# bschrag620/PyRad

Hardware: NVIDIA B200
Metric: line-gridpoint evals/s (higher is better)
Workload: dtype f32

## Files before the change

pyrad_b200/csrc/api.cu:

```cuda
#include "../../include/pyrad_b200.h"

#include <algorithm>
#include <chrono>
#include <cmath>
#include <cstdio>
#include <cstring>
#include <functional>
#include <string>
#include <vector>

#include "common.cuh"
#include "k1_prepass.cuh"
#include "k2_line_sum.cuh"
#include "k2_narrow.cuh"
#include "k2_point.cuh"
#include "k3_stream.cuh"
#include "k4_derived.cuh"
#include "k5_ingest.cuh"
#include "k9_peaks.cuh"
#include <cub/cub.cuh>
#include <thrust/iterator/counting_iterator.h>

using namespace prb;

// ... 118 lines not shown
    DevBuf<double> far_lag2[2];
    float far_delta2[2][K2_FAR_NODES] = {};
    int64_t narrow_wm = 100;
    bool batch_layers = true;
    bool k3_tma = true;
    bool point_kernel = true;
    bool fuse_single = true;
    bool split_tiles = false;
    DevBuf<double> part_sums;
    DevBuf<unsigned int> part_count;
    int64_t rec_budget_mb = 0;
    PeerState peer;
    DevBuf<unsigned int> peer_err;
    IngestScratch ingest;
    DevBuf<int2> tile_bounds_buf[2];
    int tile_bounds_next = 0;
    int extra_launches = 0;
    cudaStream_t copy_stream = nullptr, stream2 = nullptr;
    std::vector<cudaEvent_t> pipe_ev;
    unsigned long long *pin_scal = nullptr;
    DevBuf<unsigned long long> dev_scal;
    unsigned char *blk_h = nullptr;
    size_t blk_cap = 0;
    DevBuf<unsigned char> blk_d;
    K2Layer *ring_h = nullptr;
    DevBuf<K2Layer> ring_d;
    cudaEvent_t ring_ev[RING] = {};
    int ring_next = 0;

    XscTable xsc[K2_MAX_XSC];
// ... 114 lines not shown
    cudaSetDevice(e->device);
    cudaStreamSynchronize(e->stream);
    e->nu0.release(); e->s296.release(); e->gair.release(); e->gself.release();
    e->elower.release(); e->nair.release(); e->delta.release(); e->group.release(); e->einstein_a.release();
    e->idx.release(); e->recA.release(); e->recB.release(); e->recD.release(); e->gp.release(); e->st.release();
    e->out64.release(); e->scratch_a.release(); e->scratch_b.release(); e->scratch_c.release();
    e->scratch_d.release(); e->scratch_w.release();
    e->kmat.release(); e->rad.release(); e->trans.release(); e->fold.release();
    e->flux_layers.release(); e->flux_part.release(); e->flux_out.release(); e->flux_rows.release();
    e->band_part.release(); e->band_out.release(); e->band_tab.release();
    e->k2tab.release(); e->ring_d.release(); e->peer_err.release();
    if (e->blk_h) cudaFreeHost(e->blk_h);
    if (e->read_stage) cudaFreeHost(e->read_stage);
    e->blk_d.release();
    e->ingest.release();
    e->tile_bounds_buf[0].release(); e->tile_bounds_buf[1].release();
    e->far_lag[0].release(); e->far_lag[1].release(); e->far_lag2[0].release(); e->far_lag2[1].release();
    e->dev_scal.release();
    e->part_sums.release(); e->part_count.release();
    e->xsc_rows.release();
    for (auto &x : e->xsc) { x.fx.release(); x.fy.release(); }
    if (e->pin_scal) cudaFreeHost(e->pin_scal);
    for (auto x : e->pipe_ev) cudaEventDestroy(x);
    if (e->copy_stream) cudaStreamDestroy(e->copy_stream);
    if (e->stream2) cudaStreamDestroy(e->stream2);
    if (e->ring_h) { cudaFreeHost(e->ring_h); for (auto x : e->ring_ev) if (x) cudaEventDestroy(x); }
    peer_release(e);
    for (auto x : e->ev) cudaEventDestroy(x);
    cudaStreamDestroy(e->stream);
    delete e;
    return PRB_OK;
// ... 406 lines not shown

static void fill_k1_row(const prb_engine *e, const LayerJob &j, K1Layer &t) {
    const size_t na = (size_t)e->n_alloc;
    t.T = j.T; t.P = j.P;
    t.lc = layer_consts(j.T, j.P, e->res);
    t.scale = j.scale;
    t.scale_dev = j.scale_dev;
    t.wm = (double)j.wm;
    t.gp = j.gp_dev;
    t.recA = e->recA.p + na * j.slot;
    t.recB = e->recB.p + na * j.slot;
    t.recD = e->recD.p + na * j.slot;
    t.st = j.st_dev;
    t.narrow = j.narrow;
    t.pad = 0;
}

static int run_prepass(prb_engine *e, const LayerJob *jobs, int n, DebugOut dbg, int *launches = nullptr) {
    for (int k0 = 0; k0 < n; k0 += K1_MAX_LAYERS) {
        const int m = std::min(n - k0, K1_MAX_LAYERS);
        K1Table &tab = e->k1_host;
        tab.n = m;
        tab.pad = 0;
        int64_t l0 = jobs[k0].l0, l1 = jobs[k0].l1;
        for (int k = 0; k < m; ++k) {
            fill_k1_row(e, jobs[k0 + k], tab.rows[k]);
            l0 = std::min(l0, jobs[k0 + k].l0);
            l1 = std::max(l1, jobs[k0 + k].l1);
        }
        const int64_t kb = l0 & ~int64_t(3);
        const int64_t ke = std::min<int64_t>(l1 + 8, e->n_alloc);
        const int64_t cnt = ke - kb;
        if (cnt > 0) {
            LinesSoA L{e->nu0.p, e->s296.p, e->gair.p, e->gself.p, e->elower.p, e->nair.p, e->delta.p,
                       e->has_group ? e->group.p : nullptr};
            k1_prepass<false><<<(unsigned)((cnt + 255) / 256), 256, 0, e->stream>>>(L, e->idx.p, tab, kb, ke, e->n_lines,
                                                                            e->i_begin, dbg);
            CK(cudaGetLastError());
            if (launches) ++*launches;
            LineRangeTable lr;
            lr.n = 0; lr.pad = 0;
            const size_t na = (size_t)e->n_alloc;
            for (int k = 0; k < m; ++k) {
                const LayerJob &j = jobs[k0 + k];
                if (!j.filter) continue;
                LineRangeRow &r = lr.rows[lr.n++];
                r.recA = e->recA.p + na * j.slot;
                r.recB = e->recB.p + na * j.slot;
                r.recD = e->recD.p + na * j.slot;
                r.lo = j.nu_lo; r.hi = j.nu_hi;
                r.narrow = j.narrow; r.pad = 0;
            }
// ... 58 lines not shown
    CK(cudaMemsetAsync(st.p, 0, sizeof(DevState), e->stream));
    DevBuf<float4> r4, r5; DevBuf<float> r2;
    CK(r4.ensure(na)); CK(r5.ensure(na)); CK(r2.ensure(na));
    K1Table &tab = e->k1_host;
    tab.n = 1;
    K1Layer &row = tab.rows[0];
    row.T = e->last.T; row.P = e->last.P;
    row.lc = layer_consts(e->last.T, e->last.P, e->res);
    row.scale = e->last.scale;
    row.scale_dev = nullptr;
    row.wm = (double)e->last.wm;
    row.gp = e->gp.p;
    row.recA = r4.p; row.recB = r5.p; row.recD = r2.p;
    row.st = st.p;
    row.narrow = 0; row.pad = 0;
    LinesSoA L{e->nu0.p, e->s296.p, e->gair.p, e->gself.p, e->elower.p, e->nair.p, e->delta.p,
               e->has_group ? e->group.p : nullptr};
    k1_prepass<true><<<(unsigned)((na + 255) / 256), 256, 0, e->stream>>>(L, e->idx.p, tab, 0, na, n, e->i_begin, dbg);
    CK(cudaGetLastError());
    if (nu_shift) CK(cudaMemcpyAsync(nu_shift, e->scratch_a.p, sizeof(double) * n, cudaMemcpyDeviceToHost, e->stream));
    if (gamma_l) CK(cudaMemcpyAsync(gamma_l, e->scratch_b.p, sizeof(double) * n, cudaMemcpyDeviceToHost, e->stream));
    if (gamma_d) CK(cudaMemcpyAsync(gamma_d, e->scratch_c.p, sizeof(double) * n, cudaMemcpyDeviceToHost, e->stream));
    if (s_t) CK(cudaMemcpyAsync(s_t, e->scratch_d.p, sizeof(double) * n, cudaMemcpyDeviceToHost, e->stream));
    if (regime) CK(cudaMemcpyAsync(regime, reg.p, sizeof(int32_t) * n, cudaMemcpyDeviceToHost, e->stream));
    std::vector<int32_t> h_idx(index ? n : 0);
    if (index && n) CK(cudaMemcpyAsync(h_idx.data(), e->idx.p, sizeof(int32_t) * n, cudaMemcpyDeviceToHost, e->stream));
    CK(cudaStreamSynchronize(e->stream));
    if (index) for (int64_t i = 0; i < n; ++i) index[i] = h_idx[i];
    r4.release(); r5.release(); r2.release(); reg.release(); st.release();
    return PRB_OK;
// ... 71 lines not shown
    const size_t cnt = (size_t)b.n_layers * b.n_tiles;
    if (e->tile_bounds_buf[e->tile_bounds_next].ensure(cnt) != cudaSuccess)
        return fail(PRB_ERR_CUDA, "tile bounds allocation failed");
    int2 *buf = e->tile_bounds_buf[e->tile_bounds_next].p;
    e->tile_bounds_next ^= 1;
    k2_tile_bounds<<<dim3((unsigned)((b.n_tiles + 255) / 256), (unsigned)b.n_layers), 256, 0, e->stream>>>(
        b.layers, b.n_layers, b.idx, b.i_begin, b.n_tiles, KP_TILE, buf);
    CK(cudaGetLastError());
    ++e->extra_launches;
    b.tile_bounds = buf;
    return PRB_OK;
}

static void xsc_args(const prb_engine *e, K2Args &a);
static int run_line_sum(prb_engine *e, const LayerJob *jobs, int n, const K2Layer *tab_dev, int out_mode,
                        const K2Fuse *fuse, bool with_xsc = false) {
    if (n <= 0) return PRB_OK;
    K2Args a{};
    if (with_xsc) xsc_args(e, a);
    a.layers = tab_dev;
    a.n_layers = n;
    a.idx = e->idx.p;
    a.i_begin = e->i_begin;
    a.n_chunk = (int)chunk_len(e);
    a.variant = e->k2_variant;
    a.out_mode = out_mode;
    a.st = jobs[0].st_dev;
    if (fuse) a.fuse = *fuse;
    cudaError_t ce;
    if (jobs[0].narrow == 2) {
        a.n_tiles = (a.n_chunk + KP_TILE - 1) / KP_TILE;
// ... 11 lines not shown
    }
    if (jobs[0].narrow) {
        a.n_tiles = (a.n_chunk + KN_TILE - 1) / KN_TILE;
        for (int k0 = 0; k0 < n && a.n_tiles > 0; k0 += 65535) {
            K2Args b = a;
            b.layers = tab_dev + k0;
            b.n_layers = std::min(n - k0, 65535);
            int rc2 = tile_bounds(e, b);
            if (rc2) return rc2;
            k2_narrow<<<dim3((unsigned)a.n_tiles, (unsigned)b.n_layers), KN_THREADS, sizeof(KNSmem), e->stream>>>(b);
        }
        ce = cudaGetLastError();
        if (ce != cudaSuccess) return fail(PRB_ERR_CUDA, std::string("k2_narrow launch failed: ") + cudaGetErrorString(ce));
        return PRB_OK;
    }
    switch (jobs[0].ppt) {
        case 2: ce = launch_k2_t<2>(e, a); break;
        case 4: ce = launch_k2_t<4>(e, a); break;
        case 16: ce = launch_k2_t<16>(e, a); break;
        default: ce = launch_k2_t<8>(e, a); break;
    }
    if (ce != cudaSuccess) return fail(PRB_ERR_CUDA, std::string("k2_line_sum launch failed: ") + cudaGetErrorString(ce));
    return PRB_OK;
}

extern "C" int prb_line_sum_dev(prb_engine *e, void *out_dev, int out_mode) {
    if (!e) return fail(PRB_ERR_ARG, "null engine");
    if (!e->last.valid) return fail(PRB_ERR_STATE, "prb_line_sum: run prb_layer_prepass first");
    if (!e->seg.empty()) return fail(PRB_ERR_STATE, "prb_line_sum: grouped line list -- use prb_line_sum_groups");
    if (!out_dev) return fail(PRB_ERR_ARG, "prb_line_sum_dev: NULL output");
// ... 482 lines not shown
        for (int sidx = 0; sidx < pipe->S; ++sidx) {
            if (sidx + 1 < pipe->S && (rc = pipe->enqueue_piece(sidx + 1))) return rc;
            cudaStream_t st = (sidx & 1) ? pipe->stream2 : e->stream;
            CK(cudaStreamWaitEvent(st, pipe->ev[sidx], 0));
            if (sidx) CK(cudaStreamWaitEvent(st, pipe->ev_k1[sidx - 1], 0));
            const int64_t a = sidx ? pipe->line_hi[sidx - 1] : 0;
            const int64_t b = sidx == pipe->S - 1 ? na : pipe->line_hi[sidx];
            if (b > a) {
                k0_line_index<<<(unsigned)((b - a + 255) / 256), 256, 0, st>>>(e->nu0.p, n, a, b, e->range_min, e->res, e->idx.p);
                CK(cudaGetLastError());
                LayerJob jj = jobs[0];
                jj.l0 = a;
                jj.l1 = std::min<int64_t>(b, n);
                K1Table &tab = e->k1_host;
                tab.n = 1;
                tab.pad = 0;
                fill_k1_row(e, jj, tab.rows[0]);
                LinesSoA Ls{e->nu0.p, e->s296.p, e->gair.p, e->gself.p, e->elower.p, e->nair.p, e->delta.p,
                            e->has_group ? e->group.p : nullptr};
                k1_prepass<false><<<(unsigned)((b - a + 255) / 256), 256, 0, st>>>(Ls, e->idx.p, tab, a, b, n, e->i_begin, DebugOut{});
                CK(cudaGetLastError());
                launches += 2;
            }
            CK(cudaEventRecord(pipe->ev_k1[sidx], st));
            K2Args ka{};
            ka.layers = k2_dev + sidx;
            ka.n_layers = 1;
            ka.idx = e->idx.p;
            ka.i_begin = e->i_begin;
            ka.n_chunk = (int)nc;
            ka.variant = e->k2_variant;
// ... 7 lines not shown
            switch (jobs[0].ppt) {
                case 2: ce = launch_k2_sub<2>(e, ka, st); break;
                case 4: ce = launch_k2_sub<4>(e, ka, st); break;
                case 16: ce = launch_k2_sub<16>(e, ka, st); break;
                default: ce = launch_k2_sub<8>(e, ka, st); break;
            }
            if (ce != cudaSuccess) return fail(PRB_ERR_CUDA, std::string("k2_line_sum sub-launch failed: ") + cudaGetErrorString(ce));
            ++launches;
        }
        CK(cudaEventRecord(pipe->ev_k1[pipe->S], pipe->stream2));
        CK(cudaStreamWaitEvent(e->stream, pipe->ev_k1[pipe->S], 0));
    }
    for (int bi = 0; bi < (pipe ? 0 : n_batches); ++bi) {
        const int b0 = (int)(bi * slots), b1 = (int)std::min<int64_t>(n_layers, b0 + slots);
        if (e->timing) CK(cudaEventRecord(e->ev[3 * bi], e->stream));
        rc = run_prepass(e, jobs.data() + b0, b1 - b0, DebugOut{}, &launches);
        if (rc) return rc;
        if (e->timing) CK(cudaEventRecord(e->ev[3 * bi + 1], e->stream));
        for (int c0 = b0; c0 < b1;) {
            int c1 = c0 + 1;
            while (c1 < b1 && jobs[c1].narrow == jobs[c0].narrow && (jobs[c0].narrow || jobs[c1].ppt == jobs[c0].ppt)) ++c1;
            rc = run_line_sum(e, jobs.data() + c0, c1 - c0, k2_dev + c0, PRB_OUT_F32, fused ? &fuse : nullptr, true);
            if (rc) return rc;
            ++launches;
            c0 = c1;
        }
        if (e->timing) CK(cudaEventRecord(e->ev[3 * bi + 2], e->stream));
    }
    if (e->timing) CK(cudaEventRecord(e->ev[3 * n_batches], e->stream));
    if (nc > 0 && !fused) {
        if (e->k3_tma && n_layers >= K3T_LAYERS) {
            const int64_t n_strips = (nc + K3T_STRIP - 1) / K3T_STRIP;
            const int grid = (int)std::min<int64_t>(n_strips, K3T_MINB * (int64_t)e->prop.multiProcessorCount);
            double t_max = t_surface, t_min = t_surface;
            for (int l = 0; l < n_layers; ++l) { t_max = std::max(t_max, t_layer[l]); t_min = std::min(t_min, t_layer[l]); }
            double nu_min = std::max(3 * dx * std::sqrt(6.0 / 8e-7), 0.26 * t_max / c2);
            if ((3 * dx) * (3 * dx) / 8 * (c2 / t_min) * (c2 / t_min) > 1e-7) nu_min = 1e30;
// ... 887 lines not shown
```

pyrad_b200/csrc/common.cuh:

```cuda
#pragma once
#include <cuda_runtime.h>
#include <stdint.h>
#include <math.h>

namespace prb {

constexpr double kBoltz = 1.38064852E-23;
constexpr double cLight = 299792458.0;
constexpr double hPlanck = 6.62607004e-34;
constexpr double kPi = 3.141592653589793;
constexpr double kT0 = 296.0;
constexpr double kP0 = 1013.25;
constexpr double kAvogadro = 6.022140857E23;

constexpr int REGIME_GAUSS = 0, REGIME_LORENTZ = 1, REGIME_VOIGT = 2;

struct GroupParams {
    double conc;
    double dopp;
    double qratio;
    double weight;
};

struct DevState {
    unsigned int reserved0;
    unsigned int flags;
    unsigned int tile_counter;
    unsigned int pad;
};

constexpr unsigned int FLAG_OVERFLOW = 1u, FLAG_NONFINITE = 2u;

#ifndef PRB_K2_CONSUMERS
#define PRB_K2_CONSUMERS 8
#endif
#ifndef PRB_K2_ACC_SMEM
#define PRB_K2_ACC_SMEM 0
#endif
constexpr int K2_CONSUMERS = PRB_K2_CONSUMERS;
constexpr int K2_THREADS = 32 * (K2_CONSUMERS + 1);
#ifndef PRB_K2_CHUNK
#define PRB_K2_CHUNK 768
#endif
#ifndef PRB_K2_STAGES
#define PRB_K2_STAGES 3
#endif
#ifndef PRB_K2_MIN_CTAS
#define PRB_K2_MIN_CTAS 2
#endif
constexpr int K2_CHUNK = PRB_K2_CHUNK;
constexpr int K2_STAGES = PRB_K2_STAGES;
constexpr int K2_MIN_CTAS = PRB_K2_MIN_CTAS;
constexpr int K2_FLUSH = 64;
constexpr float K2_SENTINEL = 3.0e38f;

__device__ __forceinline__ uint32_t smem_u32(const void *p) {
    return (uint32_t)__cvta_generic_to_shared(p);
}
__device__ __forceinline__ void mbar_init(uint64_t *bar, uint32_t count) {
    asm volatile("mbarrier.init.shared::cta.b64 [%0], %1;" ::"r"(smem_u32(bar)), "r"(count) : "memory");
}
__device__ __forceinline__ void mbar_expect_tx(uint64_t *bar, uint32_t bytes) {
    asm volatile("mbarrier.arrive.expect_tx.shared::cta.b64 _, [%0], %1;" ::"r"(smem_u32(bar)), "r"(bytes)
                 : "memory");
}
__device__ __forceinline__ void mbar_arrive(uint64_t *bar) {
    asm volatile("mbarrier.arrive.shared::cta.b64 _, [%0];" ::"r"(smem_u32(bar)) : "memory");
}
__device__ __forceinline__ void mbar_wait(uint64_t *bar, uint32_t parity) {
    asm volatile(
        "{\n"
        ".reg .pred p;\n"
        "WAIT_%=:\n"
        "mbarrier.try_wait.parity.shared::cta.b64 p, [%0], %1;\n"
        "@p bra DONE_%=;\n"
        "bra WAIT_%=;\n"
        "DONE_%=:\n"
        "}\n" ::"r"(smem_u32(bar)),
        "r"(parity)
        : "memory");
}
__device__ __forceinline__ void mbar_wait_parked(uint64_t *bar, uint32_t parity) {
    asm volatile(
        "{\n"
        ".reg .pred p;\n"
        "WAITP_%=:\n"
        "mbarrier.try_wait.parity.shared::cta.b64 p, [%0], %1, %2;\n"
        "@p bra DONEP_%=;\n"
        "bra WAITP_%=;\n"
        "DONEP_%=:\n"
        "}\n" ::"r"(smem_u32(bar)),
        "r"(parity), "r"(4000u)
        : "memory");
}
__device__ __forceinline__ void tma_bulk_g2s(void *dst, const void *src, uint32_t bytes, uint64_t *bar) {
    asm volatile(
        "cp.async.bulk.shared::cluster.global.mbarrier::complete_tx::bytes [%0], [%1], %2, [%3];" ::"r"(
            smem_u32(dst)),
        "l"(src), "r"(bytes), "r"(smem_u32(bar))
        : "memory");
}

}
```

pyrad_b200/csrc/k1_prepass.cuh:

```cuda
#pragma once
#include "common.cuh"

namespace prb {

struct LinesSoA {
    const double *nu0, *s296, *gair, *gself, *elower, *nair, *delta;
    const int32_t *group;
};

struct LayerConsts {
    double log_t0_over_t;
    double inv_t_minus_inv_t0;
    double inv_res2;
    double res2;
    double p_over_p0;
    double neg_c2_over_t;
    double neg_c2_over_t0;
};

struct DebugOut {
    double *nu_shift, *gl, *gd, *st;
    int32_t *regime;
};

// ... 72 lines not shown

__device__ __forceinline__ double pow5(double x) { double x2 = x * x; return x2 * x2 * x; }

struct K1Layer {
    double T, P;
    LayerConsts lc;
    double scale;
    const double *scale_dev;
    double wm;
    const GroupParams *gp;
    float4 *recA, *recB;
    float *recD;
    DevState *st;
    int narrow;
    int pad;
};

constexpr int K1_MAX_LAYERS = 128;
enum K1Const {
    K1C_EXP_INV = 0, K1C_EXP_MAGIC, K1C_EXP_HI, K1C_EXP_LO, K1C_EXP_5, K1C_EXP_4, K1C_EXP_3,
    K1C_T7, K1C_T6, K1C_T5, K1C_T4, K1C_T3,
    K1C_V1, K1C_V2, K1C_V3, K1C_V4,
    K1C_E1, K1C_E2, K1C_E3,
    K1C_LOG2E, K1C_INV_SQRTPI, K1C_INV_PI, K1C_FIFTH, K1C_C2, K1C_NEG_C2_T0,
    K1C_LO_A, K1C_LO_B, K1C_HI_A, K1C_HI_B,
    K1C_BIG, K1C_COUNT
};
struct K1Table {
    int n;
    int pad;
    double c[K1C_COUNT];
    K1Layer rows[K1_MAX_LAYERS];
};
inline void k1_fill_constants(K1Table &t) {
    const double eps = 1e-14, c2 = cLight * hPlanck * 100 / kBoltz;
    const double v[K1C_COUNT] = {
        92.33248261689366, 6755399441055744.0, -0.01083042469326756, -2.9815858269852933e-12, 1.0 / 120.0, 1.0 / 24.0, 1.0 / 6.0,
        1.0 / 5040, 1.0 / 720, 1.0 / 120, 1.0 / 24, 1.0 / 6,
        2.69269, 2.42843, 4.47163, .07842,
        1.36603, .47719, .11116,
        1.4426950408889634, 0.5641895835477563, 1.0 / kPi, 0.2, c2, -c2 / kT0,
        .01 * (1 - eps), .01 * (1 + eps), 100 * (1 + eps), 100 * (1 - eps),
        8.0e37};
    for (int i = 0; i < K1C_COUNT; ++i) t.c[i] = v[i];
}
// ... 54 lines not shown
    p = fma(p, x, c[K1C_T5]);
    p = fma(p, x, c[K1C_T4]);
    p = fma(p, x, c[K1C_T3]);
    p = fma(p, x, 0.5);
    p = fma(p, x, 1.0);
    return fma(p, x, 1.0);
}

#ifndef PRB_K1_UNROLL
#define PRB_K1_UNROLL 1
#endif
constexpr int K1_UNROLL = PRB_K1_UNROLL;
#ifndef PRB_K1_MINB
#define PRB_K1_MINB 4
#endif
template <bool DEBUG = false>
__global__ void __launch_bounds__(256, PRB_K1_MINB)
k1_prepass(LinesSoA L, const int32_t *__restrict__ idx, const __grid_constant__ K1Table tab,
           int64_t l_begin, int64_t l_end, int64_t n_lines, int64_t i_base, DebugOut dbg) {
    __shared__ double exp_tab[64];
    if (threadIdx.x < 64) exp_tab[threadIdx.x] = K1_EXP_TAB[threadIdx.x];
    __syncthreads();
    const double *__restrict__ cst = tab.c;
    const double c2 = cst[K1C_C2];
    const int64_t l = l_begin + (int64_t)blockIdx.x * blockDim.x + threadIdx.x;
    const bool in_range = l < l_end;
    const bool real = in_range && l < n_lines && !(L.group && L.group[l] < 0);
    double nu = 0, delta = 0, gair = 0, gself = 0, nair = 0, elower = 0, s296 = 0;
    float nf = 0.f;
    int g = 0;
    if (real) {
        nu = L.nu0[l]; delta = L.delta[l]; gair = L.gair[l]; gself = L.gself[l];
        nair = L.nair[l]; elower = L.elower[l]; s296 = L.s296[l];
        g = L.group ? L.group[l] : 0;
        nf = -(float)((double)((int64_t)idx[l] - i_base));
    }
    const bool bad_line = real && !isfinite(nu + delta + gair + gself + nair + elower + s296);
    const double e296 = exp_k1(cst[K1C_NEG_C2_T0] * nu, exp_tab, cst);
    const double neg_c2_e = -c2 * elower;
    const int n_layers = tab.n;
// ... 149 lines not shown
```

pyrad_b200/csrc/k2_line_sum.cuh:

```cuda
#pragma once
#include "common.cuh"
#include "k3_stream.cuh"

namespace prb {

__device__ __forceinline__ float rcp_approx(float x) {
    float r;
    asm("rcp.approx.ftz.f32 %0, %1;" : "=f"(r) : "f"(x));
    return r;
}
__device__ __forceinline__ float ex2_approx(float x) {
    float r;
    asm("ex2.approx.ftz.f32 %0, %1;" : "=f"(r) : "f"(x));
    return r;
}

__device__ __forceinline__ void tma_bulk_s2g(void *dst, const void *src, uint32_t bytes) {
    asm volatile("cp.async.bulk.global.shared::cta.bulk_group [%0], [%1], %2;" ::"l"(dst), "r"(smem_u32(src)), "r"(bytes)
                 : "memory");
}
__device__ __forceinline__ void consumer_barrier() {
    asm volatile("bar.sync 1, %0;" ::"n"(K2_CONSUMERS * 32) : "memory");
}

__device__ __forceinline__ int warp_lower_bound(const int32_t *__restrict__ idx, int lo, int hi, long long key) {
    const int lane = threadIdx.x & 31;
    while (hi > lo) {
        const int span = hi - lo;
        const int step = (span + 31) >> 5;
        int pos = lo + (lane + 1) * step - 1;
        pos = pos < hi - 1 ? pos : hi - 1;
        const bool less = (long long)__ldg(idx + pos) < key;
        const unsigned m = __ballot_sync(0xffffffffu, less);
        const int c = __popc(m);
        int nlo = lo, nhi = hi;
        if (c > 0) { int p = lo + c * step - 1; p = p < hi - 1 ? p : hi - 1; nlo = p + 1; }
        if (c < 32) { int p = lo + (c + 1) * step - 1; p = p < hi - 1 ? p : hi - 1; nhi = p; }
        lo = nlo;
        hi = nhi;
    }
    return lo;
}

constexpr int K2_MAX_XSC = 8;
struct K2Layer {
    const float4 *recA;
    const float4 *recB;
    const float *recD;
    void *out;
    double inv_scale;
    int l_begin, l_end;
    int wm;
    int pad;
    double xsc_w[K2_MAX_XSC];
};

// ... 7 lines not shown
    long long n_total;
    double x0, dx, x_last;
    float *rad[K2_MAX_DST];
    float *trans[K2_MAX_DST];
};

struct K2Args {
    const K2Layer *layers;
    int n_layers;
    const int32_t *idx;
    long long i_begin;
    int n_chunk;
    int n_tiles;
    int tile_base;
    const int2 *tile_bounds;
    int variant;
    int out_mode;
    DevState *st;
    K2Fuse fuse;
    const double *far_lag;
    float far_delta[16];
    const double *far_lag2;
    float far_delta2[16];
    const double *xsc_sigma;
    long long xsc_ld;
    int n_xsc;
    int parts;
    double *part_sums;
    unsigned int *part_count;
};
// ... 16 lines not shown
#define PRB_K2_FAR2_ENABLE 1
#endif
constexpr bool K2_FAR2 = PRB_K2_FAR2_ENABLE != 0;
constexpr int K2_FAR2_MIN_DOMAINS = 4;
static_assert(K2_CONSUMERS % K2_FAR2_SPANS == 0, "a tile is a whole number of level-2 domains");

struct K2Desc {
    int tile0;
    int cnt;
    int flags;
    int layer;
    int part;
};
constexpr int K2_FIRST = 1, K2_LAST = 2, K2_END = 4;

struct K2Smem {
    float4 rA[K2_STAGES][K2_CHUNK];
    float4 rB[K2_STAGES][K2_CHUNK];
    float rD[K2_STAGES][K2_CHUNK];
    K2Desc desc[K2_STAGES];
    uint64_t full[K2_STAGES];
    uint64_t empty[K2_STAGES];
    double far2[2][K2_CONSUMERS][K2_FAR_NODES];
    double2 faracc[2][K2_CONSUMERS * 32];
    int part_last;
};

template <int P>
__host__ __device__ constexpr size_t K2_SMEM_BASE() {
    return ((sizeof(K2Smem) + (PRB_K2_ACC_SMEM ? sizeof(double) * P * K2_CONSUMERS * 32 : 0)) + 127) & ~size_t(127);
}
template <int P>
__host__ __device__ constexpr size_t K2_SMEM_BYTES(bool peer_staging) {
    return K2_SMEM_BASE<P>() + (peer_staging ? sizeof(float) * 2 * K2_CONSUMERS * 32 * P : 0);
}

template <int H>
// ... 227 lines not shown
#pragma unroll
            for (int h = 0; h < H; ++h) {
                const float ex = s.fi[h].x + a.x, ey = s.fi[h].y + a.x;
                const float e2x = ex * ex, e2y = ey * ey;
                float tx = a.z * rcp_approx(e2x + b.x), ty = a.z * rcp_approx(e2y + b.x);
                tx = fmaf(b.z, ex2_approx(b.w * e2x), tx);
                ty = fmaf(b.z, ex2_approx(b.w * e2y), ty);
                s.a32[h].x += (fabsf(ex) <= wmf) ? tx : 0.f;
                s.a32[h].y += (fabsf(ey) <= wmf) ? ty : 0.f;
            }
        }
        s.flush();
    }
}

template <int P, bool FAR, bool SPLIT>
__device__ __forceinline__ void k2_line_sum_body(const K2Args &a) {
    static_assert(P >= 2 && P % 2 == 0, "points per thread must be even (packed FP32x2)");
    static_assert(!FAR || P == 4 || P == 8, "far-field tables exist for 128- and 256-point spans");
    constexpr int H = P / 2;
    constexpr int TILE = K2_CONSUMERS * 32 * P;
    constexpr int SPAN = 32 * P;
    extern __shared__ __align__(128) unsigned char smem_raw[];
    K2Smem &sm = *reinterpret_cast<K2Smem *>(smem_raw);
    const int tid = threadIdx.x, lane = tid & 31, warp = tid >> 5;

    if (tid == 0) {
        for (int s = 0; s < K2_STAGES; ++s) {
            mbar_init(&sm.full[s], 1);
            mbar_init(&sm.empty[s], K2_CONSUMERS);
        }
        asm volatile("fence.mbarrier_init.release.cluster;" ::: "memory");
        asm volatile("fence.proxy.async.shared::cta;" ::: "memory");
    }
    __syncthreads();

    if (warp == K2_CONSUMERS) {
        uint32_t it = 0;
        auto slot_acquire = [&](uint32_t &stage) {
            stage = it % K2_STAGES;
            mbar_wait_parked(&sm.empty[stage], ((it / K2_STAGES) & 1) ^ 1);
        };
        const int parts = (SPLIT && a.parts > 1) ? a.parts : 1;
        const int n_items = a.n_layers * a.n_tiles * parts;
        while (true) {
            int item = 0;
            if (lane == 0) item = (int)atomicAdd(&a.st->tile_counter, 1u);
            item = __shfl_sync(0xffffffffu, item, 0);
            if (item >= n_items) break;
            const int n_lt = a.n_layers * a.n_tiles;
            const int pidx = item / n_lt;
            const int lt = item - pidx * n_lt;
            const int half = parts >> 1, step = pidx >> 2, r = pidx & 3;
            const int part = parts < 4 ? pidx : (r == 0 ? half - 1 - step : r == 1 ? half + step : r == 2 ? step : parts - 1 - step);
            const int layer = lt / a.n_tiles;
            const int tile = a.tile_base + lt - layer * a.n_tiles;
            const K2Layer *L = a.layers + layer;
            const int wm = __ldg(&L->wm), l_begin = __ldg(&L->l_begin), l_end = __ldg(&L->l_end);
            const float4 *recA = L->recA;
            const float4 *recB = L->recB;
            const float *recD = L->recD;
            const int tile0 = tile * TILE;
            const long long k_lo = a.i_begin + tile0 - wm;
            const long long k_hi = a.i_begin + tile0 + TILE - 1 + wm + 1;
            int lo = warp_lower_bound(a.idx, l_begin, l_end, k_lo);
            const int hi = warp_lower_bound(a.idx, lo, l_end, k_hi);
            lo &= ~3;
            const int nch = hi > lo ? (hi - lo + K2_CHUNK - 1) / K2_CHUNK : 1;
            const int c0 = (int)((long long)part * nch / parts), c1 = (int)((long long)(part + 1) * nch / parts);
            const int cn = c1 > c0 ? c1 - c0 : 1;
            for (int k = 0; k < cn; ++k, ++it) {
                const int c = c0 + k;
                uint32_t stage;
                slot_acquire(stage);
                if (lane == 0) {
                    const int first = lo + c * K2_CHUNK;
                    const int cnt = c1 > c0 ? max(min(K2_CHUNK, hi - first), 0) : 0;
                    sm.desc[stage] = K2Desc{tile0, cnt, (k == 0 ? K2_FIRST : 0) | (k == cn - 1 ? K2_LAST : 0), layer, part};
                    if (cnt > 0) {
                        const uint32_t ce = (uint32_t)((cnt + 3) & ~3);
                        mbar_expect_tx(&sm.full[stage], ce * 36u);
                        tma_bulk_g2s(sm.rA[stage], recA + first, ce * 16u, &sm.full[stage]);
                        tma_bulk_g2s(sm.rB[stage], recB + first, ce * 16u, &sm.full[stage]);
                        tma_bulk_g2s(sm.rD[stage], recD + first, ce * 4u, &sm.full[stage]);
                    } else {
                        mbar_arrive(&sm.full[stage]);
                    }
                }
                __syncwarp();
            }
        }
        uint32_t stage;
        slot_acquire(stage);
        if (lane == 0) {
            sm.desc[stage] = K2Desc{0, 0, K2_END, 0, 0};
            mbar_arrive(&sm.full[stage]);
        }
        return;
    }

    float wmf = 0.f;
    Acc<H> s;
#pragma unroll
    for (int h = 0; h < H; ++h) { s.a32[h] = make_float2(0.f, 0.f); s.fi[h] = make_float2(0.f, 0.f); }
#if PRB_K2_ACC_SMEM
    s.a64 = reinterpret_cast<double *>(smem_raw + sizeof(K2Smem)) + tid;
#endif
#pragma unroll
    for (int p = 0; p < P; ++p) s.acc(p) = 0.0;
    int wb = 0;
    float wbf = 0.f, we1f = 0.f;
    double2 *far = &sm.faracc[0][tid];
    double2 *far2 = &sm.faracc[1][tid];
    float dbf = 0.f;
// ... 108 lines not shown
                b4 = __reduce_add_sync(0xffffffffu, c4);
                const int b5 = __reduce_add_sync(0xffffffffu, c5);
                bg0 = __reduce_add_sync(0xffffffffu, cg0);
                bg1 = __reduce_add_sync(0xffffffffu, cg1);
                lorentz_paired<H, true>(sA, sB, b0, b1, wmf, s);
                lorentz_paired<H, false>(sA, sB, b1, b4, wmf, s);
                lorentz_paired<H, true>(sA, sB, b4, b5, wmf, s);
            }
            if (dgmax > 0.f) {
                gauss_pass<H, true>(sA, sB, sD, bg0, min(bg1, b1), wbf, we1f, wmf, s);
                gauss_pass<H, false>(sA, sB, sD, max(bg0, b1), min(bg1, b4), wbf, we1f, wmf, s);
                gauss_pass<H, true>(sA, sB, sD, max(bg0, b4), bg1, wbf, we1f, wmf, s);
            }
        }
        __syncwarp();
        if (lane == 0) mbar_arrive(&sm.empty[stage]);

        if (d.flags & K2_LAST) {
            const K2Layer *L = a.layers + d.layer;
            const double inv_scale = __ldg(&L->inv_scale);
            void *out = L->out;
            const bool bulk = a.fuse.enabled && a.fuse.n_dst > 1 && d.tile0 + TILE <= a.n_chunk;
            float *stage_rad = reinterpret_cast<float *>(smem_raw + K2_SMEM_BASE<P>());
            float *stage_tr = stage_rad + TILE;
            if (bulk) {
                if (tid == 0) asm volatile("cp.async.bulk.wait_group.read 0;" ::: "memory");
                consumer_barrier();
            }
            if (FAR) {
                double v0 = far->x, v1 = far->y, w0 = far2->x, w1 = far2->y;
#pragma unroll
// ... 113 lines not shown
```

Baseline: 4989 billion.

## Remove dedicated producer warp and precompute tile line bounds in prepass

Drops the dedicated TMA producer warp from the line-sum kernel. The last consumer warp to release a stage now refills it, with shared-memory counters and an ordered issue ticket replacing the empty mbarriers. Per-tile line-index bounds for wide layers are computed by extra blocks of the prepass kernel and stored in a device buffer, so the refill path reads them instead of doing a warp binary search. This frees a warp per CTA and takes the search off the critical path, but refill latency now lands on consumer warps and the spin on the issue counter can serialize them.

Measured after the change: 5056 billion (median of 6 runs). 1.4% higher.

```diff
diff --git a/pyrad_b200/csrc/api.cu b/pyrad_b200/csrc/api.cu
--- a/pyrad_b200/csrc/api.cu
+++ b/pyrad_b200/csrc/api.cu
@@ -156,6 +156,7 @@
     DevBuf<unsigned int> peer_err;
     IngestScratch ingest;
     DevBuf<int2> tile_bounds_buf[2];
+    DevBuf<int2> k2_bounds;
     int tile_bounds_next = 0;
     int extra_launches = 0;
     cudaStream_t copy_stream = nullptr, stream2 = nullptr;
@@ -300,7 +301,7 @@
     if (e->read_stage) cudaFreeHost(e->read_stage);
     e->blk_d.release();
     e->ingest.release();
-    e->tile_bounds_buf[0].release(); e->tile_bounds_buf[1].release();
+    e->tile_bounds_buf[0].release(); e->tile_bounds_buf[1].release(); e->k2_bounds.release();
     e->far_lag[0].release(); e->far_lag[1].release(); e->far_lag2[0].release(); e->far_lag2[1].release();
     e->dev_scal.release();
     e->part_sums.release(); e->part_count.release();
@@ -737,28 +738,43 @@
     t.st = j.st_dev;
     t.narrow = j.narrow;
     t.pad = 0;
-}
-
-static int run_prepass(prb_engine *e, const LayerJob *jobs, int n, DebugOut dbg, int *launches = nullptr) {
+    t.bounds = nullptr;
+    t.b_tiles = t.b_tile_pts = t.b_l_begin = t.b_l_end = t.b_wm = 0;
+}
+
+static int run_prepass(prb_engine *e, const LayerJob *jobs, int n, DebugOut dbg, int *launches = nullptr,
+                       int2 *bounds = nullptr, int64_t bounds_ld = 0) {
+    const int64_t nc = chunk_len(e);
     for (int k0 = 0; k0 < n; k0 += K1_MAX_LAYERS) {
         const int m = std::min(n - k0, K1_MAX_LAYERS);
         K1Table &tab = e->k1_host;
         tab.n = m;
-        tab.pad = 0;
+        tab.bounds_blocks = 0;
         int64_t l0 = jobs[k0].l0, l1 = jobs[k0].l1;
         for (int k = 0; k < m; ++k) {
-            fill_k1_row(e, jobs[k0 + k], tab.rows[k]);
-            l0 = std::min(l0, jobs[k0 + k].l0);
-            l1 = std::max(l1, jobs[k0 + k].l1);
+            const LayerJob &j = jobs[k0 + k];
+            K1Layer &r = tab.rows[k];
+            fill_k1_row(e, j, r);
+            l0 = std::min(l0, j.l0);
+            l1 = std::max(l1, j.l1);
+            if (bounds && !j.narrow) {
+                r.bounds = bounds + (size_t)(k0 + k) * bounds_ld;
+                r.b_tile_pts = K2_CONSUMERS * 32 * j.ppt;
+                r.b_tiles = (int)((nc + r.b_tile_pts - 1) / r.b_tile_pts);
+                r.b_l_begin = (int)j.l0;
+                r.b_l_end = (int)j.l1;
+                r.b_wm = (int)j.wm;
+                tab.bounds_blocks = std::max(tab.bounds_blocks, (r.b_tiles + 7) / 8);
+            }
         }
         const int64_t kb = l0 & ~int64_t(3);
-        const int64_t ke = std::min<int64_t>(l1 + 8, e->n_alloc);
+        const int64_t ke = std::max(kb, std::min<int64_t>(l1 + 8, e->n_alloc));
         const int64_t cnt = ke - kb;
-        if (cnt > 0) {
+        if (cnt > 0 || tab.bounds_blocks > 0) {
             LinesSoA L{e->nu0.p, e->s296.p, e->gair.p, e->gself.p, e->elower.p, e->nair.p, e->delta.p,
                        e->has_group ? e->group.p : nullptr};
-            k1_prepass<false><<<(unsigned)((cnt + 255) / 256), 256, 0, e->stream>>>(L, e->idx.p, tab, kb, ke, e->n_lines,
-                                                                            e->i_begin, dbg);
+            const int64_t blocks = (cnt + 255) / 256 + (int64_t)m * tab.bounds_blocks;
+            k1_prepass<false><<<(unsigned)blocks, 256, 0, e->stream>>>(L, e->idx.p, tab, kb, ke, e->n_lines, e->i_begin, dbg);
             CK(cudaGetLastError());
             if (launches) ++*launches;
             LineRangeTable lr;
@@ -847,6 +863,8 @@
     row.recA = r4.p; row.recB = r5.p; row.recD = r2.p;
     row.st = st.p;
     row.narrow = 0; row.pad = 0;
+    row.bounds = nullptr;
+    tab.bounds_blocks = 0;
     LinesSoA L{e->nu0.p, e->s296.p, e->gair.p, e->gself.p, e->elower.p, e->nair.p, e->delta.p,
                e->has_group ? e->group.p : nullptr};
     k1_prepass<true><<<(unsigned)((na + 255) / 256), 256, 0, e->stream>>>(L, e->idx.p, tab, 0, na, n, e->i_begin, dbg);
@@ -948,7 +966,8 @@
 
 static void xsc_args(const prb_engine *e, K2Args &a);
 static int run_line_sum(prb_engine *e, const LayerJob *jobs, int n, const K2Layer *tab_dev, int out_mode,
-                        const K2Fuse *fuse, bool with_xsc = false) {
+                        const K2Fuse *fuse, bool with_xsc = false, const int2 *wide_bounds = nullptr,
+                        int64_t bounds_ld = 0) {
     if (n <= 0) return PRB_OK;
     K2Args a{};
     if (with_xsc) xsc_args(e, a);
@@ -990,6 +1009,8 @@
         if (ce != cudaSuccess) return fail(PRB_ERR_CUDA, std::string("k2_narrow launch failed: ") + cudaGetErrorString(ce));
         return PRB_OK;
     }
+    a.tile_bounds = wide_bounds;
+    a.bounds_ld = (int)bounds_ld;
     switch (jobs[0].ppt) {
         case 2: ce = launch_k2_t<2>(e, a); break;
         case 4: ce = launch_k2_t<4>(e, a); break;
@@ -1502,7 +1523,7 @@
                 jj.l1 = std::min<int64_t>(b, n);
                 K1Table &tab = e->k1_host;
                 tab.n = 1;
-                tab.pad = 0;
+                tab.bounds_blocks = 0;
                 fill_k1_row(e, jj, tab.rows[0]);
                 LinesSoA Ls{e->nu0.p, e->s296.p, e->gair.p, e->gself.p, e->elower.p, e->nair.p, e->delta.p,
                             e->has_group ? e->group.p : nullptr};
@@ -1540,13 +1561,16 @@
     for (int bi = 0; bi < (pipe ? 0 : n_batches); ++bi) {
         const int b0 = (int)(bi * slots), b1 = (int)std::min<int64_t>(n_layers, b0 + slots);
         if (e->timing) CK(cudaEventRecord(e->ev[3 * bi], e->stream));
-        rc = run_prepass(e, jobs.data() + b0, b1 - b0, DebugOut{}, &launches);
+        const int64_t bounds_ld = (nc + 511) / 512;
+        CK(e->k2_bounds.ensure((size_t)std::max<int64_t>(bounds_ld, 1) * (b1 - b0)));
+        rc = run_prepass(e, jobs.data() + b0, b1 - b0, DebugOut{}, &launches, e->k2_bounds.p, bounds_ld);
         if (rc) return rc;
         if (e->timing) CK(cudaEventRecord(e->ev[3 * bi + 1], e->stream));
         for (int c0 = b0; c0 < b1;) {
             int c1 = c0 + 1;
             while (c1 < b1 && jobs[c1].narrow == jobs[c0].narrow && (jobs[c0].narrow || jobs[c1].ppt == jobs[c0].ppt)) ++c1;
-            rc = run_line_sum(e, jobs.data() + c0, c1 - c0, k2_dev + c0, PRB_OUT_F32, fused ? &fuse : nullptr, true);
+            rc = run_line_sum(e, jobs.data() + c0, c1 - c0, k2_dev + c0, PRB_OUT_F32, fused ? &fuse : nullptr, true,
+                              e->k2_bounds.p + (size_t)(c0 - b0) * bounds_ld, bounds_ld);
             if (rc) return rc;
             ++launches;
             c0 = c1;
diff --git a/pyrad_b200/csrc/common.cuh b/pyrad_b200/csrc/common.cuh
--- a/pyrad_b200/csrc/common.cuh
+++ b/pyrad_b200/csrc/common.cuh
@@ -38,7 +38,7 @@
 #define PRB_K2_ACC_SMEM 0
 #endif
 constexpr int K2_CONSUMERS = PRB_K2_CONSUMERS;
-constexpr int K2_THREADS = 32 * (K2_CONSUMERS + 1);
+constexpr int K2_THREADS = 32 * K2_CONSUMERS;
 #ifndef PRB_K2_CHUNK
 #define PRB_K2_CHUNK 768
 #endif
@@ -53,6 +53,25 @@
 constexpr int K2_MIN_CTAS = PRB_K2_MIN_CTAS;
 constexpr int K2_FLUSH = 64;
 constexpr float K2_SENTINEL = 3.0e38f;
+
+__device__ __forceinline__ int warp_lower_bound(const int32_t *__restrict__ idx, int lo, int hi, long long key) {
+    const int lane = threadIdx.x & 31;
+    while (hi > lo) {
+        const int span = hi - lo;
+        const int step = (span + 31) >> 5;
+        int pos = lo + (lane + 1) * step - 1;
+        pos = pos < hi - 1 ? pos : hi - 1;
+        const bool less = (long long)__ldg(idx + pos) < key;
+        const unsigned m = __ballot_sync(0xffffffffu, less);
+        const int c = __popc(m);
+        int nlo = lo, nhi = hi;
+        if (c > 0) { int p = lo + c * step - 1; p = p < hi - 1 ? p : hi - 1; nlo = p + 1; }
+        if (c < 32) { int p = lo + (c + 1) * step - 1; p = p < hi - 1 ? p : hi - 1; nhi = p; }
+        lo = nlo;
+        hi = nhi;
+    }
+    return lo;
+}
 
 __device__ __forceinline__ uint32_t smem_u32(const void *p) {
     return (uint32_t)__cvta_generic_to_shared(p);
@@ -80,19 +99,6 @@
         "r"(parity)
         : "memory");
 }
-__device__ __forceinline__ void mbar_wait_parked(uint64_t *bar, uint32_t parity) {
-    asm volatile(
-        "{\n"
-        ".reg .pred p;\n"
-        "WAITP_%=:\n"
-        "mbarrier.try_wait.parity.shared::cta.b64 p, [%0], %1, %2;\n"
-        "@p bra DONEP_%=;\n"
-        "bra WAITP_%=;\n"
-        "DONEP_%=:\n"
-        "}\n" ::"r"(smem_u32(bar)),
-        "r"(parity), "r"(4000u)
-        : "memory");
-}
 __device__ __forceinline__ void tma_bulk_g2s(void *dst, const void *src, uint32_t bytes, uint64_t *bar) {
     asm volatile(
         "cp.async.bulk.shared::cluster.global.mbarrier::complete_tx::bytes [%0], [%1], %2, [%3];" ::"r"(
diff --git a/pyrad_b200/csrc/k1_prepass.cuh b/pyrad_b200/csrc/k1_prepass.cuh
--- a/pyrad_b200/csrc/k1_prepass.cuh
+++ b/pyrad_b200/csrc/k1_prepass.cuh
@@ -110,6 +110,9 @@
     DevState *st;
     int narrow;
     int pad;
+    int2 *bounds;
+    int b_tiles, b_tile_pts;
+    int b_l_begin, b_l_end, b_wm;
 };
 
 constexpr int K1_MAX_LAYERS = 128;
@@ -124,7 +127,7 @@
 };
 struct K1Table {
     int n;
-    int pad;
+    int bounds_blocks;
     double c[K1C_COUNT];
     K1Layer rows[K1_MAX_LAYERS];
 };
@@ -209,16 +212,31 @@
 #ifndef PRB_K1_MINB
 #define PRB_K1_MINB 4
 #endif
+__device__ __noinline__ void k1_tile_bounds(const K1Table &tab, const int32_t *__restrict__ idx, int64_t i_base, int b) {
+    const K1Layer &R = tab.rows[b / tab.bounds_blocks];
+    const int t = (b % tab.bounds_blocks) * 8 + (int)(threadIdx.x >> 5);
+    if (!R.bounds || t >= R.b_tiles) return;
+    const long long tile0 = i_base + (long long)t * R.b_tile_pts;
+    const int lo = warp_lower_bound(idx, R.b_l_begin, R.b_l_end, tile0 - R.b_wm);
+    const int hi = warp_lower_bound(idx, lo, R.b_l_end, tile0 + R.b_tile_pts - 1 + R.b_wm + 1);
+    if ((threadIdx.x & 31) == 0) R.bounds[t] = make_int2(lo, hi);
+}
+
 template <bool DEBUG = false>
 __global__ void __launch_bounds__(256, PRB_K1_MINB)
 k1_prepass(LinesSoA L, const int32_t *__restrict__ idx, const __grid_constant__ K1Table tab,
            int64_t l_begin, int64_t l_end, int64_t n_lines, int64_t i_base, DebugOut dbg) {
+    const int bounds_blocks = tab.n * tab.bounds_blocks;
+    if ((int)blockIdx.x < bounds_blocks) {
+        k1_tile_bounds(tab, idx, i_base, (int)blockIdx.x);
+        return;
+    }
     __shared__ double exp_tab[64];
     if (threadIdx.x < 64) exp_tab[threadIdx.x] = K1_EXP_TAB[threadIdx.x];
     __syncthreads();
     const double *__restrict__ cst = tab.c;
     const double c2 = cst[K1C_C2];
-    const int64_t l = l_begin + (int64_t)blockIdx.x * blockDim.x + threadIdx.x;
+    const int64_t l = l_begin + (int64_t)(blockIdx.x - bounds_blocks) * blockDim.x + threadIdx.x;
     const bool in_range = l < l_end;
     const bool real = in_range && l < n_lines && !(L.group && L.group[l] < 0);
     double nu = 0, delta = 0, gair = 0, gself = 0, nair = 0, elower = 0, s296 = 0;
diff --git a/pyrad_b200/csrc/k2_line_sum.cuh b/pyrad_b200/csrc/k2_line_sum.cuh
--- a/pyrad_b200/csrc/k2_line_sum.cuh
+++ b/pyrad_b200/csrc/k2_line_sum.cuh
@@ -21,25 +21,6 @@
 }
 __device__ __forceinline__ void consumer_barrier() {
     asm volatile("bar.sync 1, %0;" ::"n"(K2_CONSUMERS * 32) : "memory");
-}
-
-__device__ __forceinline__ int warp_lower_bound(const int32_t *__restrict__ idx, int lo, int hi, long long key) {
-    const int lane = threadIdx.x & 31;
-    while (hi > lo) {
-        const int span = hi - lo;
-        const int step = (span + 31) >> 5;
-        int pos = lo + (lane + 1) * step - 1;
-        pos = pos < hi - 1 ? pos : hi - 1;
-        const bool less = (long long)__ldg(idx + pos) < key;
-        const unsigned m = __ballot_sync(0xffffffffu, less);
-        const int c = __popc(m);
-        int nlo = lo, nhi = hi;
-        if (c > 0) { int p = lo + c * step - 1; p = p < hi - 1 ? p : hi - 1; nlo = p + 1; }
-        if (c < 32) { int p = lo + (c + 1) * step - 1; p = p < hi - 1 ? p : hi - 1; nhi = p; }
-        lo = nlo;
-        hi = nhi;
-    }
-    return lo;
 }
 
 constexpr int K2_MAX_XSC = 8;
@@ -77,6 +58,7 @@
     int n_tiles;
     int tile_base;
     const int2 *tile_bounds;
+    int bounds_ld;
     int variant;
     int out_mode;
     DevState *st;
@@ -123,13 +105,23 @@
 };
 constexpr int K2_FIRST = 1, K2_LAST = 2, K2_END = 4;
 
+struct K2Cursor {
+    int layer, part, tile0;
+    int lo, hi;
+    int c0, c1;
+    int k, cn;
+    int done;
+};
+
 struct K2Smem {
     float4 rA[K2_STAGES][K2_CHUNK];
     float4 rB[K2_STAGES][K2_CHUNK];
     float rD[K2_STAGES][K2_CHUNK];
     K2Desc desc[K2_STAGES];
     uint64_t full[K2_STAGES];
-    uint64_t empty[K2_STAGES];
+    unsigned int released[K2_STAGES];
+    unsigned int issued;
+    K2Cursor cur;
     double far2[2][K2_CONSUMERS][K2_FAR_NODES];
     double2 faracc[2][K2_CONSUMERS * 32];
     int part_last;
@@ -387,6 +379,78 @@
     }
 }
 
+struct K2Item {
+    int part, layer, tile;
+};
+__device__ __forceinline__ K2Item k2_item(const K2Args &a, int item, int parts) {
+    const int n_lt = a.n_layers * a.n_tiles;
+    const int pidx = item / n_lt;
+    const int lt = item - pidx * n_lt;
+    const int half = parts >> 1, step = pidx >> 2, r = pidx & 3;
+    const int part = parts < 4 ? pidx : (r == 0 ? half - 1 - step : r == 1 ? half + step : r == 2 ? step : parts - 1 - step);
+    const int layer = lt / a.n_tiles;
+    return K2Item{part, layer, a.tile_base + lt - layer * a.n_tiles};
+}
+
+template <int TILE, bool SPLIT>
+__device__ __forceinline__ void k2_refill(K2Smem &sm, const K2Args &a, uint32_t stage) {
+    const int lane = threadIdx.x & 31;
+    K2Cursor c = sm.cur;
+    if (c.done) return;
+    if (c.k == c.cn) {
+        const int parts = (SPLIT && a.parts > 1) ? a.parts : 1;
+        int item = 0;
+        if (lane == 0) item = (int)atomicAdd(&a.st->tile_counter, 1u);
+        item = __shfl_sync(0xffffffffu, item, 0);
+        if (item >= a.n_layers * a.n_tiles * parts) {
+            if (lane == 0) {
+                sm.desc[stage] = K2Desc{0, 0, K2_END, 0, 0};
+                mbar_arrive(&sm.full[stage]);
+                sm.cur.done = 1;
+            }
+            __syncwarp();
+            return;
+        }
+        const K2Item w = k2_item(a, item, parts);
+        const int tile0 = w.tile * TILE;
+        int lo, hi;
+        if (a.tile_bounds) {
+            const int2 bd = __ldg(a.tile_bounds + (size_t)w.layer * a.bounds_ld + (w.tile - a.tile_base));
+            lo = bd.x;
+            hi = bd.y;
+        } else {
+            const K2Layer *L = a.layers + w.layer;
+            const int wm = __ldg(&L->wm), l_begin = __ldg(&L->l_begin), l_end = __ldg(&L->l_end);
+            const long long k_lo = a.i_begin + tile0 - wm;
+            const long long k_hi = a.i_begin + tile0 + TILE - 1 + wm + 1;
+            lo = warp_lower_bound(a.idx, l_begin, l_end, k_lo);
+            hi = warp_lower_bound(a.idx, lo, l_end, k_hi);
+        }
+        lo &= ~3;
+        const int nch = hi > lo ? (hi - lo + K2_CHUNK - 1) / K2_CHUNK : 1;
+        const int c0 = (int)((long long)w.part * nch / parts), c1 = (int)((long long)(w.part + 1) * nch / parts);
+        c = K2Cursor{w.layer, w.part, tile0, lo, hi, c0, c1, 0, c1 > c0 ? c1 - c0 : 1, 0};
+    }
+    if (lane == 0) {
+        const int first = c.lo + (c.c0 + c.k) * K2_CHUNK;
+        const int cnt = c.c1 > c.c0 ? max(min(K2_CHUNK, c.hi - first), 0) : 0;
+        sm.desc[stage] = K2Desc{c.tile0, cnt, (c.k == 0 ? K2_FIRST : 0) | (c.k == c.cn - 1 ? K2_LAST : 0), c.layer, c.part};
+        if (cnt > 0) {
+            const K2Layer *L = a.layers + c.layer;
+            const uint32_t ce = (uint32_t)((cnt + 3) & ~3);
+            mbar_expect_tx(&sm.full[stage], ce * 36u);
+            tma_bulk_g2s(sm.rA[stage], L->recA + first, ce * 16u, &sm.full[stage]);
+            tma_bulk_g2s(sm.rB[stage], L->recB + first, ce * 16u, &sm.full[stage]);
+            tma_bulk_g2s(sm.rD[stage], L->recD + first, ce * 4u, &sm.full[stage]);
+        } else {
+            mbar_arrive(&sm.full[stage]);
+        }
+        ++c.k;
+        sm.cur = c;
+    }
+    __syncwarp();
+}
+
 template <int P, bool FAR, bool SPLIT>
 __device__ __forceinline__ void k2_line_sum_body(const K2Args &a) {
     static_assert(P >= 2 && P % 2 == 0, "points per thread must be even (packed FP32x2)");
@@ -398,79 +462,21 @@
     K2Smem &sm = *reinterpret_cast<K2Smem *>(smem_raw);
     const int tid = threadIdx.x, lane = tid & 31, warp = tid >> 5;
 
-    if (tid == 0) {
-        for (int s = 0; s < K2_STAGES; ++s) {
-            mbar_init(&sm.full[s], 1);
-            mbar_init(&sm.empty[s], K2_CONSUMERS);
-        }
-        asm volatile("fence.mbarrier_init.release.cluster;" ::: "memory");
-        asm volatile("fence.proxy.async.shared::cta;" ::: "memory");
+    if (warp == 0) {
+        if (lane == 0) {
+            for (int s = 0; s < K2_STAGES; ++s) {
+                mbar_init(&sm.full[s], 1);
+                sm.released[s] = 0;
+            }
+            sm.issued = K2_STAGES;
+            sm.cur = K2Cursor{0, 0, 0, 0, 0, 0, 0, 0, 0, 0};
+            asm volatile("fence.mbarrier_init.release.cluster;" ::: "memory");
+            asm volatile("fence.proxy.async.shared::cta;" ::: "memory");
+        }
+        __syncwarp();
+        for (int s = 0; s < K2_STAGES; ++s) k2_refill<TILE, SPLIT>(sm, a, s);
     }
     __syncthreads();
-
-    if (warp == K2_CONSUMERS) {
-        uint32_t it = 0;
-        auto slot_acquire = [&](uint32_t &stage) {
-            stage = it % K2_STAGES;
-            mbar_wait_parked(&sm.empty[stage], ((it / K2_STAGES) & 1) ^ 1);
-        };
-        const int parts = (SPLIT && a.parts > 1) ? a.parts : 1;
-        const int n_items = a.n_layers * a.n_tiles * parts;
-        while (true) {
-            int item = 0;
-            if (lane == 0) item = (int)atomicAdd(&a.st->tile_counter, 1u);
-            item = __shfl_sync(0xffffffffu, item, 0);
-            if (item >= n_items) break;
-            const int n_lt = a.n_layers * a.n_tiles;
-            const int pidx = item / n_lt;
-            const int lt = item - pidx * n_lt;
-            const int half = parts >> 1, step = pidx >> 2, r = pidx & 3;
-            const int part = parts < 4 ? pidx : (r == 0 ? half - 1 - step : r == 1 ? half + step : r == 2 ? step : parts - 1 - step);
-            const int layer = lt / a.n_tiles;
-            const int tile = a.tile_base + lt - layer * a.n_tiles;
-            const K2Layer *L = a.layers + layer;
-            const int wm = __ldg(&L->wm), l_begin = __ldg(&L->l_begin), l_end = __ldg(&L->l_end);
-            const float4 *recA = L->recA;
-            const float4 *recB = L->recB;
-            const float *recD = L->recD;
-            const int tile0 = tile * TILE;
-            const long long k_lo = a.i_begin + tile0 - wm;
-            const long long k_hi = a.i_begin + tile0 + TILE - 1 + wm + 1;
-            int lo = warp_lower_bound(a.idx, l_begin, l_end, k_lo);
-            const int hi = warp_lower_bound(a.idx, lo, l_end, k_hi);
-            lo &= ~3;
-            const int nch = hi > lo ? (hi - lo + K2_CHUNK - 1) / K2_CHUNK : 1;
-            const int c0 = (int)((long long)part * nch / parts), c1 = (int)((long long)(part + 1) * nch / parts);
-            const int cn = c1 > c0 ? c1 - c0 : 1;
-            for (int k = 0; k < cn; ++k, ++it) {
-                const int c = c0 + k;
-                uint32_t stage;
-                slot_acquire(stage);
-                if (lane == 0) {
-                    const int first = lo + c * K2_CHUNK;
-                    const int cnt = c1 > c0 ? max(min(K2_CHUNK, hi - first), 0) : 0;
-                    sm.desc[stage] = K2Desc{tile0, cnt, (k == 0 ? K2_FIRST : 0) | (k == cn - 1 ? K2_LAST : 0), layer, part};
-                    if (cnt > 0) {
-                        const uint32_t ce = (uint32_t)((cnt + 3) & ~3);
-                        mbar_expect_tx(&sm.full[stage], ce * 36u);
-                        tma_bulk_g2s(sm.rA[stage], recA + first, ce * 16u, &sm.full[stage]);
-                        tma_bulk_g2s(sm.rB[stage], recB + first, ce * 16u, &sm.full[stage]);
-                        tma_bulk_g2s(sm.rD[stage], recD + first, ce * 4u, &sm.full[stage]);
-                    } else {
-                        mbar_arrive(&sm.full[stage]);
-                    }
-                }
-                __syncwarp();
-            }
-        }
-        uint32_t stage;
-        slot_acquire(stage);
-        if (lane == 0) {
-            sm.desc[stage] = K2Desc{0, 0, K2_END, 0, 0};
-            mbar_arrive(&sm.full[stage]);
-        }
-        return;
-    }
 
     float wmf = 0.f;
     Acc<H> s;
@@ -609,7 +615,23 @@
             }
         }
         __syncwarp();
-        if (lane == 0) mbar_arrive(&sm.empty[stage]);
+        unsigned int last = 0;
+        if (lane == 0) {
+            __threadfence_block();
+            last = atomicAdd(&sm.released[stage], 1u) == (it / K2_STAGES + 1) * K2_CONSUMERS - 1;
+            if (last) {
+                while (*reinterpret_cast<volatile unsigned int *>(&sm.issued) != it + K2_STAGES) {}
+                __threadfence_block();
+            }
+        }
+        if (__shfl_sync(0xffffffffu, last, 0)) {
+            __syncwarp();
+            k2_refill<TILE, SPLIT>(sm, a, stage);
+            if (lane == 0) {
+                __threadfence_block();
+                *reinterpret_cast<volatile unsigned int *>(&sm.issued) = it + K2_STAGES + 1;
+            }
+        }
 
         if (d.flags & K2_LAST) {
             const K2Layer *L = a.layers + d.layer;
```
